# brain-research/l2hmc

Hardware: AMD Instinct MI355X
Metric: chain_leapfrog_steps_per_sec (higher is better)
Workload: dtype f32

## Files before the change

l2hmc_amd/csrc/l2hmc_abi.hip:

```cpp
#include <cstdlib>
#include "traj_tile.hpp"
#include "traj_lane.hpp"

namespace l2hmc {

thread_local char g_err[512] = "";
thread_local char g_kernel[96] = "";
void note_kernel(const char* fmt, long long a, long long b, long long c, long long d) { snprintf(g_kernel, sizeof(g_kernel), fmt, a, b, c, d); }

int fail(int code, const char* fmt, const char* a, long long b, long long c) {
  snprintf(g_err, sizeof(g_err), fmt, a, b, c);
  return code;
}

__global__ void pack_net_kernel(L2hmcNet net, int d, int H, int KH, int NT, float* out) {
  const int idx = blockIdx.x * blockDim.x + threadIdx.x;
  const int ngf = net_groups(NT) * 256;
  if (idx >= net_floats(NT)) return;
  float val = 0.f;
  if (idx < ngf) {
    const int g = idx >> 8, lane = (idx >> 2) & 63, r = idx & 3;
    const int i = lane & 15, q = lane >> 4;
    const int ui = ((i & 3) < KH) ? (i >> 2) * KH + (i & 3) : -1;
    const int uk = (r < KH) ? q * KH + r : -1;
// ... 292 lines not shown
  if (NW > 1 && (k.ekind == L2HMC_ENERGY_GAUSS_DENSE || k.ekind == L2HMC_ENERGY_GMM || lr))
    o += 16LL * k.xb_stride;
  k.o_red = (int)o;
  o += (long long)NW * 16 * 8;
  const int nc = k.ekind == L2HMC_ENERGY_GMM ? k.ncomp : 1;
  k.o_mu = (int)o;
  o += (long long)nc * DP;
  k.o_prec = (int)o;
  if (k.ekind == L2HMC_ENERGY_GAUSS_DIAG) o += DP;
  if ((k.ekind == L2HMC_ENERGY_GAUSS_DENSE || k.ekind == L2HMC_ENERGY_GMM) && !wg)
    o += (long long)nc * gauss_floats(NT);
  if (lr && NW > 1) o += (long long)NW * NT * 256;
  k.o_logc = (int)o;
  o += round4(nc);
  if (lr) {
    const long long need = logistic_floats(k.ncomp, k.d);
    const char* env = getenv("L2HMC_LOGISTIC_LDS");
    k.easy = !(env != nullptr && env[0] == '0') && (o + need + kLadLds) * 4 <= kMaxLdsBytes;
    if (k.easy) {
      k.o_mu = (int)o;
      o += need;
    }
  }
  return o * 4;
}

long long plan_lds_fast(KArgs& k, int NW, int DT, bool f16) {
  const int NT = k.NT, DP = 16 * NT, NTp = NW * DT;
  long long o = 0;
  k.o_fw = (int)o;
  o += 2LL * fast_fw_net(NTp, f16);
  k.o_fc = (int)o;
  o += 2LL * fast_fc_net(NTp);
  k.o_rec = (int)o;
  o += 2LL * fast_rec_dir(NTp, k.T);
  k.o_P = (int)o;
  if (NW > 1) o += 2LL * NW * 256;
  k.xb_stride = DP + 4;
  k.o_XB = (int)o;
  if (NW > 1 && (k.ekind == L2HMC_ENERGY_GAUSS_DENSE || k.ekind == L2HMC_ENERGY_GMM)) o += 16LL * k.xb_stride;
  k.o_red = (int)o;
  o += (long long)NW * 16 * 8;
  const int nc = k.ekind == L2HMC_ENERGY_GMM ? k.ncomp : 1;
  k.o_mu = (int)o;
  o += (long long)nc * DP;
  k.o_prec = (int)o;
  if (k.ekind == L2HMC_ENERGY_GAUSS_DIAG) o += DP;
  if (k.ekind == L2HMC_ENERGY_GAUSS_DENSE || k.ekind == L2HMC_ENERGY_GMM) o += (long long)nc * gauss_floats(NT);
  k.o_logc = (int)o;
  o += round4(nc);
  return o * 4;
}

long long plan_lds_tile(KArgs& k, int DT) {
  long long o = 0;
  k.o_fw = (int)o;
  o += 2LL * tile_fw_net(DT);
  k.o_state = (int)o;
  o += tile_l1_floats(DT);
  k.o_fc = (int)o;
  o += 2LL * fast_fc_net(DT);
  k.o_rec = (int)o;
  o += 2LL * fast_rec_dir(DT, k.T);
  k.o_mu = (int)o;
  o += 16LL * DT;
  k.o_prec = (int)o;
  o += 16LL * DT;
  k.o_logc = (int)o;
  return o * 4;
}

int check_energy(const L2hmcEnergy* e, int d) {
  if (e == nullptr) return fail(L2HMC_ERR_ARG, "energy is NULL%s");
  switch (e->kind) {
    case L2HMC_ENERGY_GAUSS_DIAG:
    case L2HMC_ENERGY_GAUSS_DENSE:
      if (!e->mu || !e->prec) return fail(L2HMC_ERR_ARG, "gaussian energy needs mu and prec%s");
      break;
    case L2HMC_ENERGY_GMM:
      if (!e->mu || !e->prec || !e->logc || e->n_comp < 1)
        return fail(L2HMC_ERR_ARG, "gmm energy needs mu, prec, logc, n_comp >= 1%s");
      break;
    case L2HMC_ENERGY_ROUGHWELL:
      if (!(e->eta > 0.f)) return fail(L2HMC_ERR_ARG, "roughwell needs eta > 0%s");
      break;
    case L2HMC_ENERGY_FUNNEL:
      if (!(e->eta > 0.f) || d < 2) return fail(L2HMC_ERR_ARG, "funnel needs sigma > 0 and d >= 2%s");
      break;
    case L2HMC_ENERGY_LOGISTIC:
      if (!e->mu) return fail(L2HMC_ERR_ARG, "logistic regression needs the packed data (mu, l2hmc_pack_logistic)%s");
      if (e->n_comp < 1 || e->n_comp > kLogisticMaxRows)
        return fail(L2HMC_ERR_ARG, "logistic regression needs 1 <= n_comp = n_data <= 1048576 (got %s%lld)", "", e->n_comp);
      if (d > kLogisticMaxDim) return fail(L2HMC_ERR_ARG, "logistic regression supports d <= 128 (got %s%lld)", "", d);
      if (!(e->eta > 0.f) || !(e->eta <= 3.402823466e38f))
        return fail(L2HMC_ERR_ARG, "logistic regression needs eta = prior variance sigma^2 > 0 and finite%s");
      break;
    default:
      return fail(L2HMC_ERR_ARG, "unknown energy kind %s%lld", "", e->kind);
  }
  if (!(e->temperature > 0.f)) return fail(L2HMC_ERR_ARG, "temperature must be > 0%s");
  if (!(e->anneal_beta >= 0.f && e->anneal_beta <= 1.f)) return fail(L2HMC_ERR_ARG, "anneal_beta must be in [0, 1] (0 = off)%s");
  return L2HMC_OK;
}

void fill_energy(KArgs& k, const L2hmcEnergy* e) {
  k.ekind = e->kind;
// ... 29 lines not shown
  if (v == 1) return false;
  NW = 4;
  DT = NT <= 8 ? 2 : (NT <= 16 ? 4 : 8);
  return NT <= 32;
}

bool pick_geometry_logistic(int d, int v, int& DT, int& NW) {
  if (d > kLogisticMaxDim || (v != 0 && v != 1 && v != 4)) return false;
  DT = tiles_of(d) <= 4 ? 1 : 2;
  NW = 4;
  if (v == 1) {
    DT = NW = 1;
    return tiles_of(d) <= 1;
  }
  return v == 0 || DT == 1;
}
bool pick_geometry_of(int ekind, int d, long long N, int v, int& DT, int& NW, int cus = 0) {
  return ekind == L2HMC_ENERGY_LOGISTIC ? pick_geometry_logistic(d, v, DT, NW) : pick_geometry(d, N, v, DT, NW, cus);
}

struct EnvOverrides {
  bool f32_mfma;
  int lane_res;
};

static EnvOverrides read_env() {
  static const bool f32 = [] { const char* e = getenv("L2HMC_F32_MFMA"); return e && e[0] && e[0] != '0'; }();
  const char* e = getenv("L2HMC_LANE_RES");
  return {f32, (e != nullptr && e[0] >= '0' && e[0] <= '2') ? e[0] - '0' : -1};
}

struct Variant {
  int value;
  int forced;
  bool all_auto;
  int geom;
  bool f32;
};

static Variant decode_variant(int variant, bool env_f32) {
  Variant v;
  v.f32 = variant >= 200 || env_f32;
  v.value = variant >= 200 ? variant - 200 : variant;
  v.forced = v.value >= 100 ? FAM_GENERAL : v.value == 32 ? FAM_LANE : v.value == 8 ? FAM_WIDE : v.value == 16 ? FAM_TILE : -1;
  v.all_auto = v.value == 0;
  v.geom = v.value >= 100 ? v.value - 100 : (v.value == 16 || v.value == 33) ? 0 : v.value;
  return v;
}

#ifndef WIDE_DENSE_MIN_NT
#define WIDE_DENSE_MIN_NT 8
#endif

static int plan_geometry(const L2hmcTrajectoryArgs& a, const Variant& v, int cus, TrajPlan& p) {
  if (!pick_geometry_of(a.energy.kind, a.d, a.n_chains, v.geom, p.DT, p.NW, cus))
    return fail(L2HMC_ERR_UNSUPPORTED, "d = %s%lld not supported with variant %lld", "", a.d, v.value);
  return L2HMC_OK;
}

static void plan_general(const L2hmcTrajectoryArgs& a, KArgs& k, TrajPlan& p) {
  p.family = FAM_GENERAL;
  p.lds = plan_lds(k, a.packed_nets != nullptr, true, p.NW, p.DT);
}

static int plan_trajectory(const L2hmcTrajectoryArgs& a, KArgs& k, int KH, int cus, const EnvOverrides& env, TrajPlan& p) {
  const Variant v = decode_variant(a.variant, env.f32_mfma);
  p = TrajPlan();
  p.ek = k.ekind;
  p.KH = KH <= 3 ? 3 : 4;
  const bool nets = a.packed_nets != nullptr, has_u = a.u != nullptr || (a.rng_flags & L2HMC_RNG_U);
  const bool plain = k.beta == 1.f && k.temperature == 1.f;
  const bool lr = k.ekind == L2HMC_ENERGY_LOGISTIC;
  if (lr && (v.forced == FAM_LANE || v.forced == FAM_WIDE || v.forced == FAM_TILE))
    return fail(L2HMC_ERR_UNSUPPORTED, "variant %s%lld: the logistic-regression target runs on the general kernel only (variant 0 or 100 + v)",
                "", v.value);
  if (lr) {
    int rc = plan_geometry(a, v, cus, p);
    if (rc) return rc;
    plan_general(a, k, p);
    return L2HMC_OK;
  }
  const bool lane_able = nets && a.ais_beta == nullptr && plain && k.n_steps >= 1 && lane_supported(k.ekind, a.d, a.H, k.ncomp) &&
                         (a.d <= 16 || a.x_next != nullptr || !has_u);
  if (v.forced == FAM_LANE && !lane_able)
    return fail(L2HMC_ERR_UNSUPPORTED, "variant 32 (one chain per lane) needs S/T/Q nets and a Gaussian / mixture / Rough-Well target with d <= 4%s");
  const bool lane_auto = (a.d <= 2 && a.n_chains >= 256 * cus) || (a.d <= 4 && a.n_chains >= 512 * cus);
  if (lane_able && (v.forced == FAM_LANE || (v.all_auto && lane_auto))) {
    p.family = FAM_LANE;
    p.DP = a.d <= 2 ? 2 : 4;
    p.HPR = lane_hu(a.H) == 10 ? 5 : 8;
    if (p.DP == 2 && p.HPR == 5)
      p.RES = env.lane_res >= 0 ? env.lane_res
              : k.ekind == L2HMC_ENERGY_GAUSS_DIAG ? 2
              : a.n_chains < 3LL * 64 * 1024 ? 1 : 0;
    return L2HMC_OK;
  }
  const bool wide_dense = k.ekind == L2HMC_ENERGY_GAUSS_DENSE || k.ekind == L2HMC_ENERGY_GMM;
  const bool wide_kind = k.ekind == L2HMC_ENERGY_GAUSS_DIAG || k.ekind == L2HMC_ENERGY_ROUGHWELL || wide_dense;
  const bool wide_able = nets && wide_kind && !(k.M > 1 && a.x_next == nullptr) && k.NT <= 32;
  if (v.forced == FAM_WIDE && !(wide_able && k.NT >= 4))
    return fail(L2HMC_ERR_UNSUPPORTED, "variant 8 (LDS-resident state) needs S/T/Q nets, a Gaussian or Rough-Well target, 64 <= d <= 512 and x_next when n_proposals > 1%s");
  if (wide_able && (v.forced == FAM_WIDE || (v.all_auto && k.NT > (wide_dense ? WIDE_DENSE_MIN_NT : 8)))) {
    KArgs kw = k;
    if (v.f32 || wide_dense || !plain) kw.packed16 = nullptr;
    int nw;
    const long long lds = plan_lds_wide(kw, nw);
    if (lds <= kMaxLdsBytes) {
      k = kw;
      p.family = FAM_WIDE;
      p.NW = nw;
      p.KH = KH == 3 ? 3 : 4;
      p.f16 = kw.packed16 != nullptr;
      p.lds = lds;
      return L2HMC_OK;
    }
    if (v.forced == FAM_WIDE) return fail(L2HMC_ERR_UNSUPPORTED, "variant 8: %s%lld bytes of LDS needed (T x d too large)", "", lds);
  }
  int rc = plan_geometry(a, v, cus, p);
  if (rc) return rc;
  const bool fast = nets && p.DT <= 2 && k.n_steps >= 1 && v.forced != FAM_GENERAL && plain;
  if (fast && a.d <= 4 && v.geom == 0 && k.ekind != L2HMC_ENERGY_FUNNEL && (k.ekind != L2HMC_ENERGY_GMM || k.ncomp <= 8)) {
    const long long lds = plan_lds_fast(k, 1, 1, !v.f32);
    if (lds <= kMaxLdsBytes) {
      p.family = FAM_SMALL;
      p.f16 = !v.f32;
      p.lds = lds;
      return L2HMC_OK;
    }
  }
  const bool tile_kind = k.ekind == L2HMC_ENERGY_GAUSS_DIAG || k.ekind == L2HMC_ENERGY_ROUGHWELL;
  const bool tileable = nets && tile_kind && k.NT >= 3 && k.NT <= 4 && k.n_steps >= 1 && plain && !(has_u && a.x_next == nullptr) &&
                        !v.f32;
  if (v.forced == FAM_TILE && !tileable)
    return fail(L2HMC_ERR_UNSUPPORTED, "variant 16 (one wave per tile) needs S/T/Q nets, a diagonal-Gaussian or Rough-Well target, 33 <= d <= 64 and x_next whenever u is given%s");
  if (tileable && (v.forced == FAM_TILE || (v.all_auto && a.n_chains >= 64LL * cus))) {
    const long long lds = plan_lds_tile(k, k.NT);
    if (lds <= kMaxLdsBytes) {
      p.family = FAM_TILE;
      p.DT = k.NT;
      p.tpw = (2 * lds > kMaxLdsBytes && a.n_chains >= 128LL * cus) ? 8 : 4;
      p.half = a.d - 16 * (k.NT - 1) <= 2;
      p.lds = lds;
      return L2HMC_OK;
    }
    if (v.forced == FAM_TILE)
      return fail(L2HMC_ERR_UNSUPPORTED, "variant 16: %s%lld bytes of LDS needed (T too large for the one-wave-per-tile kernel)", "", lds);
  }
  if (fast) {
    p.family = FAM_FAST;
    if (!v.f32 && tile_kind) {
      p.lds = plan_lds_fast(k, p.NW, p.DT, true);
      if (p.lds <= kMaxLdsBytes) {
        p.f16 = 1;
        return L2HMC_OK;
      }
    }
    p.lds = plan_lds_fast(k, p.NW, p.DT);
    if (p.lds <= kMaxLdsBytes) return L2HMC_OK;
  }
  plan_general(a, k, p);
  return L2HMC_OK;
}

static void note_plan(const TrajPlan& p) {
  switch (p.family) {
    case FAM_LANE:
      if (p.RES != 0) return note_kernel("traj_lane_kernel<%lld, %lld, %lld, %lld>", p.ek, p.DP, p.HPR, p.RES);
      return note_kernel("traj_lane_kernel<%lld, %lld, %lld>", p.ek, p.DP, p.HPR);
    case FAM_WIDE: return note_kernel(p.f16 ? "traj_wide_kernel<f16x2>" : "traj_wide_kernel");
    case FAM_SMALL: return note_kernel(p.f16 ? "traj_small_kernel<%lld, %lld, 1>" : "traj_small_kernel<%lld, %lld>", p.ek, p.KH);
    case FAM_TILE:
      return note_kernel(p.half ? "traj_tile_kernel<%lld, %lld, %lld, %lld, true>" : "traj_tile_kernel<%lld, %lld, %lld, %lld, false>",
                         p.ek, p.DT, p.KH, p.tpw);
    case FAM_FAST:
      return note_kernel(p.f16 ? "traj_fast_kernel<%lld, %lld, %lld, %lld, 1>" : "traj_fast_kernel<%lld, %lld, %lld, %lld>", p.ek, p.DT,
                         p.NW, p.KH);
    case FAM_LADDER: return note_kernel("traj_ladder_kernel<%lld, %lld, %lld, %lld>", p.ek, p.DT, p.NW, p.KH);
    default: return note_kernel("traj_kernel<%lld, %lld, %lld, %lld>", p.ek, p.DT, p.NW, p.KH);
  }
}

static int launch_plan(const TrajPlan& p, const KArgs& k, hipStream_t s, const LadArgs* lg = nullptr) {
  return on_energy_kind(p.ek, [&](auto ek) {
    constexpr int EK = decltype(ek)::value;
    if (p.family == FAM_LADDER) return launch_ladder_ek<EK>(p, k, *lg, s);
    if constexpr (EK != L2HMC_ENERGY_FUNNEL && EK != L2HMC_ENERGY_LOGISTIC) {
      if (p.family == FAM_LANE) return launch_lane_ek<EK>(p, k, s);
      if (p.family == FAM_WIDE) return launch_wide_ek<EK>(p, k, s);
    }
    if constexpr (EK == L2HMC_ENERGY_GAUSS_DIAG || EK == L2HMC_ENERGY_ROUGHWELL) {
      if (p.family == FAM_TILE) return launch_tile_ek<EK>(p, k, s);
      if (p.family == FAM_FAST && p.f16) return launch_fast16_ek<EK>(p, k, s);
    }
    return launch_ek<EK>(p, k, s);
  });
}

}

using namespace l2hmc;

#ifdef L2HMC_PHASE_TIMING
static unsigned long long* g_dbg = nullptr;
extern "C" void l2hmc_set_debug_buffer(void* p) { g_dbg = (unsigned long long*)p; }
#define L2HMC_DBG_PTR g_dbg
#else
#define L2HMC_DBG_PTR nullptr
#endif

extern "C" {

int l2hmc_abi_version(void) { return L2HMC_ABI_VERSION; }

int32_t l2hmc_last_kernel(char* buf, int32_t n) {
  if (!buf || n < 1) return fail(L2HMC_ERR_ARG, "l2hmc_last_kernel: bad argument%s");
  snprintf(buf, (size_t)n, "%s", g_kernel);
  return (int32_t)strlen(g_kernel);
}

const char* l2hmc_last_error(void) { return g_err; }

int64_t l2hmc_struct_bytes(int32_t which) {
  switch (which) {
    case L2HMC_STRUCT_NET: return sizeof(L2hmcNet);
    case L2HMC_STRUCT_ENERGY: return sizeof(L2hmcEnergy);
    case L2HMC_STRUCT_TRAJECTORY_ARGS: return sizeof(L2hmcTrajectoryArgs);
    case L2HMC_STRUCT_MLP3: return sizeof(L2hmcMlp3);
    case L2HMC_STRUCT_SPLIT_ARGS: return sizeof(L2hmcSplitArgs);
    case L2HMC_STRUCT_TRAIN_ARGS: return sizeof(L2hmcTrainArgs);
    case L2HMC_STRUCT_TRAIN_SPLIT_ARGS: return sizeof(L2hmcTrainSplitArgs);
    case L2HMC_STRUCT_TRAIN_STEP: return sizeof(L2hmcTrainStep);
    case L2HMC_STRUCT_LADDER_ARGS: return sizeof(L2hmcLadderArgs);
  }
  return fail(L2HMC_ERR_ARG, "l2hmc_struct_bytes: unknown struct id%s");
}

int64_t l2hmc_packed_nets_floats(int32_t d, int32_t H) {
  if (d < 1 || H < 1) return fail(L2HMC_ERR_ARG, "d and H must be >= 1%s");
  if (H > 15) return fail(L2HMC_ERR_UNSUPPORTED, "fused nets support H <= 15 (got %s%lld)", "", H);
  if (d > 512) return fail(L2HMC_ERR_UNSUPPORTED, "fused nets support d <= 512 (got %s%lld)", "", d);
  return 2LL * net_floats(tiles_of(d)) + 2LL * lane_layout(d, H).total + 2LL * net_f16_floats(tiles_of(d));
// ... 365 lines not shown
```

l2hmc_amd/csrc/l2hmc_kernels.hpp:

```cpp
#pragma once
#include <hip/hip_runtime.h>
#include <stdint.h>
#include <stdio.h>
#include <string.h>
#include <type_traits>

#include "../../include/l2hmc.h"

namespace l2hmc {

typedef float f4 __attribute__((ext_vector_type(4)));

#define MFMA16(a, b, c) __builtin_amdgcn_mfma_f32_16x16x4f32((a), (b), (c), 0, 0, 0)

__host__ __device__ constexpr bool weights_in_global(int DT) { return DT >= 4; }

int fail(int code, const char* fmt, const char* a = "", long long b = 0, long long c = 0);
inline float roughwell_den(const L2hmcEnergy* e) {
  if (e->den > 0.f) return e->den;
  return e->easy ? e->eta : (float)((double)e->eta * (double)e->eta);
}
void note_kernel(const char* fmt, long long a = 0, long long b = 0, long long c = 0, long long d = 0);
inline bool adam_args_ok(float lr, float beta1, float beta2, float epsilon, int64_t step) {
  return step >= 1 && lr >= 0.f && (beta1 >= 0.f && beta1 < 1.f) && (beta2 >= 0.f && beta2 < 1.f) && epsilon > 0.f;
// ... 854 lines not shown
  extern __shared__ __attribute__((aligned(16))) float smem[];
  lds_poison(smem);
  const int tid = threadIdx.x, lane = tid & 63;
  const int w = NW > 1 ? __builtin_amdgcn_readfirstlane(tid >> 6) : 0;
  const int c = lane & 15, q = lane >> 4;
  const long long chain = (long long)blockIdx.x * 16 + c;
  const bool live = chain < A.N;
  stage_energy<EK, weights_in_global(DT)>(A, smem, tid, 64 * NW);
  f4 x[DT], g[DT];
  load_state<DT, NW>(A.x, A, chain, live, w, q, x);
  __syncthreads();
  float U[1];
  grad_energy<EK, DT, NW>(A, smem, w, lane, x, g, U[0], true);
  store_state<DT, NW>(A.grad_out, A, chain, live, w, q, g);
  chain_allreduce<NW, 1>(U, smem + A.o_red, w, lane);
  if (A.U_out != nullptr && live && w == 0 && lane < 16) A.U_out[chain] = U[0];
}

template <int EK, int DT, int NW>
__global__ __launch_bounds__(64 * NW) void paccept_kernel(const KArgs A) {
  extern __shared__ __attribute__((aligned(16))) float smem[];
  lds_poison(smem);
  const int tid = threadIdx.x, lane = tid & 63;
  const int w = NW > 1 ? __builtin_amdgcn_readfirstlane(tid >> 6) : 0;
  const int c = lane & 15, q = lane >> 4;
  const long long chain = (long long)blockIdx.x * 16 + c;
  const bool live = chain < A.N;
  stage_energy<EK, weights_in_global(DT)>(A, smem, tid, 64 * NW);
  f4 x[DT], v[DT], g[DT];
  float red[4];
  __syncthreads();
  load_state<DT, NW>(A.x, A, chain, live, w, q, x);
  load_state<DT, NW>(A.v, A, chain, live, w, q, v);
  grad_energy<EK, DT, NW>(A, smem, w, lane, x, g, red[0], true);
  red[1] = 0.f;
#pragma unroll
  for (int t = 0; t < DT; ++t) red[1] += 0.5f * hsum(v[t] * v[t]);
  load_state<DT, NW>(A.x1, A, chain, live, w, q, x);
  load_state<DT, NW>(A.v1, A, chain, live, w, q, v);
  grad_energy<EK, DT, NW>(A, smem, w, lane, x, g, red[2], true);
  red[3] = 0.f;
#pragma unroll
  for (int t = 0; t < DT; ++t) red[3] += 0.5f * hsum(v[t] * v[t]);
  chain_allreduce<NW, 4>(red, smem + A.o_red, w, lane);
  if (live && w == 0 && lane < 16) {
    const float val = (red[0] + red[1]) - (red[2] + red[3]) + A.logjac_in[chain];
    A.p_out[chain] = accept_prob(val);
  }
}


const int kMaxLdsBytes = 160 * 1024;

enum Family { FAM_GENERAL, FAM_FAST, FAM_SMALL, FAM_TILE, FAM_WIDE, FAM_LANE, FAM_LADDER, FAM_ENERGY, FAM_PACCEPT };

struct TrajPlan {
  int family = FAM_GENERAL;
  int ek = 0;
  int DT = 1, NW = 1;
  int KH = 3;
  int tpw = 4;
  bool half = false;
  int DP = 0, HPR = 0, RES = 0;
  int f16 = 0;
  long long lds = 0;
};

template <class K, class... X>
int launch_kernel(K kern, long long blocks, int threads, long long lds_bytes, hipStream_t s, const X&... args) {
  if (lds_bytes > kMaxLdsBytes)
    return fail(L2HMC_ERR_UNSUPPORTED, "needs %s%lld bytes of LDS (> 160 KiB): d too large for the LDS-resident weight path", "", lds_bytes);
  if (lds_bytes > 48 * 1024) {
    hipError_t e = hipFuncSetAttribute(reinterpret_cast<const void*>(kern),
                                       hipFuncAttributeMaxDynamicSharedMemorySize, (int)lds_bytes);
    if (e != hipSuccess) return fail(L2HMC_ERR_HIP, "hipFuncSetAttribute: %s", hipGetErrorString(e));
  }
  if (blocks > 0x7fffffffLL) return fail(L2HMC_ERR_UNSUPPORTED, "too many chains%s");
  hipLaunchKernelGGL(kern, dim3((unsigned)blocks), dim3(threads), (size_t)lds_bytes, s, args...);
  hipError_t e = hipGetLastError();
  if (e != hipSuccess) return fail(L2HMC_ERR_HIP, "kernel launch: %s", hipGetErrorString(e));
  return L2HMC_OK;
}

template <auto V> using ic = std::integral_constant<decltype(V), V>;

template <auto A, auto B, class F>
int on_either(bool first, F&& f) { return first ? f(ic<A>{}) : f(ic<B>{}); }

template <class F>
int on_energy_kind(int ek, F&& f) {
  switch (ek) {
    case 1: return f(ic<1>{});
    case 2: return f(ic<2>{});
    case 3: return f(ic<3>{});
    case 4: return f(ic<4>{});
    case 5: return f(ic<5>{});
    case 7: return f(ic<7>{});
  }
  return fail(L2HMC_ERR_ARG, "unknown energy kind%s");
}

template <int DT_, int NW_> struct Geom { static constexpr int DT = DT_, NW = NW_; };
template <class... G> struct Geoms {};
using GeneralGeoms = Geoms<Geom<1, 1>, Geom<2, 1>, Geom<4, 1>, Geom<1, 4>, Geom<2, 4>, Geom<4, 4>, Geom<8, 4>>;
using LogisticGeoms = Geoms<Geom<1, 1>, Geom<1, 4>, Geom<2, 4>>;
using FastGeoms = Geoms<Geom<1, 1>, Geom<2, 1>, Geom<1, 4>, Geom<2, 4>, Geom<2, 2>>;

template <class... G, class F>
int on_geometry(Geoms<G...>, int DT, int NW, const char* what, F&& f) {
  int rc = L2HMC_OK;
  const bool found = ((DT == G::DT && NW == G::NW && ((rc = f(ic<G::DT>{}, ic<G::NW>{})), true)) || ...);
  return found ? rc : fail(L2HMC_ERR_UNSUPPORTED, "no %skernel for this geometry", what);
}

template <int EK>
int launch_ek(const TrajPlan& p, const KArgs& k, hipStream_t s);
template <int EK>
int launch_fast16_ek(const TrajPlan& p, const KArgs& k, hipStream_t s);
template <int EK>
int launch_tile_ek(const TrajPlan& p, const KArgs& k, hipStream_t s);
template <int EK>
int launch_ladder_ek(const TrajPlan& p, const KArgs& k, const LadArgs& l, hipStream_t s);
template <int EK>
int launch_wide_ek(const TrajPlan& p, const KArgs& k, hipStream_t s);
template <int EK>
int launch_lane_ek(const TrajPlan& p, const KArgs& k, hipStream_t s);

}
```

l2hmc_amd/csrc/traj_fast.hpp:

```cpp
#pragma once
#include "l2hmc_kernels.hpp"
#include "bf3k.hpp"


namespace l2hmc {

__device__ __forceinline__ float relu_i(float a) { return __int_as_float(max(__float_as_int(a), 0)); }
__device__ __forceinline__ f4 rcp4(f4 a) {
  return f4{__builtin_amdgcn_rcpf(a.x), __builtin_amdgcn_rcpf(a.y), __builtin_amdgcn_rcpf(a.z),
            __builtin_amdgcn_rcpf(a.w)};
}
__device__ __forceinline__ f4 ex2_4(f4 a) {
  return f4{__builtin_amdgcn_exp2f(a.x), __builtin_amdgcn_exp2f(a.y), __builtin_amdgcn_exp2f(a.z),
            __builtin_amdgcn_exp2f(a.w)};
}

typedef _Float16 h2v __attribute__((ext_vector_type(2)));
typedef _Float16 h8v __attribute__((ext_vector_type(8)));
typedef float f2v __attribute__((ext_vector_type(2)));
#define L2HMC_F16_SCALE 64.0f
struct WF16 {
  h8v a1;
  h8v a2;
};
// ... 2 lines not shown
  h2v r;
  const float ns = -L2HMC_F16_SCALE;
  asm("v_fma_mixlo_f16 %0, %1, %2, %3 op_sel:[0,0,0] op_sel_hi:[1,0,0]" : "=v"(r) : "v"(h), "s"(ns), "v"(a0));
  asm("v_fma_mixhi_f16 %0, %1, %2, %3 op_sel:[1,0,0] op_sel_hi:[1,0,0]" : "+v"(r) : "v"(h), "s"(ns), "v"(a1));
  return r;
}
template <bool LAT>
__device__ __forceinline__ h8v split16(f4 a) {
  const f4 ad = a * (1.f / L2HMC_F16_SCALE);
  const h2v h01 = cvt_pk16(ad.x, ad.y), h23 = cvt_pk16(ad.z, ad.w);
  h2v l01, l23;
  if constexpr (LAT) {
    float r0, r1, r2, r3;
    const float ns = -L2HMC_F16_SCALE;
    asm("v_fma_mix_f32 %0, %1, %2, %3 op_sel:[0,0,0] op_sel_hi:[1,0,0]" : "=v"(r0) : "v"(h01), "s"(ns), "v"(a.x));
    asm("v_fma_mix_f32 %0, %1, %2, %3 op_sel:[1,0,0] op_sel_hi:[1,0,0]" : "=v"(r1) : "v"(h01), "s"(ns), "v"(a.y));
    asm("v_fma_mix_f32 %0, %1, %2, %3 op_sel:[0,0,0] op_sel_hi:[1,0,0]" : "=v"(r2) : "v"(h23), "s"(ns), "v"(a.z));
    asm("v_fma_mix_f32 %0, %1, %2, %3 op_sel:[1,0,0] op_sel_hi:[1,0,0]" : "=v"(r3) : "v"(h23), "s"(ns), "v"(a.w));
    l01 = cvt_pk16(r0, r1);
    l23 = cvt_pk16(r2, r3);
  } else {
    l01 = lo_pair16(h01, a.x, a.y);
    l23 = lo_pair16(h23, a.z, a.w);
  }
  return h8v{h01.x, h01.y, h23.x, h23.y, l01.x, l01.y, l23.x, l23.y};
}
__device__ __forceinline__ WF16 wsplit16(f4 w) {
  const float sc = L2HMC_F16_SCALE;
  const h2v h01 = cvt_pk16(w.x, w.y), h23 = cvt_pk16(w.z, w.w);
  const f4 r = f4{w.x - (float)h01.x, w.y - (float)h01.y, w.z - (float)h23.x, w.w - (float)h23.y} * sc;
  const h2v L01 = cvt_pk16(r.x, r.y), L23 = cvt_pk16(r.z, r.w);
  const h2v H01 = cvt_pk16((float)h01.x * sc, (float)h01.y * sc), H23 = cvt_pk16((float)h23.x * sc, (float)h23.y * sc);
  const h2v l01 = cvt_pk16((float)L01.x / sc, (float)L01.y / sc), l23 = cvt_pk16((float)L23.x / sc, (float)L23.y / sc);
  WF16 f;
  f.a1 = h8v{H01.x, H01.y, H23.x, H23.y, h01.x, h01.y, h23.x, h23.y};
  f.a2 = h8v{L01.x, L01.y, L23.x, L23.y, l01.x, l01.y, l23.x, l23.y};
  return f;
}
#define L2HMC_F16_STATE_MAX 2.5e5f
__device__ __forceinline__ float amax4(f4 a) { return fmaxf(fmaxf(fabsf(a.x), fabsf(a.y)), fmaxf(fabsf(a.z), fabsf(a.w))); }
__device__ __forceinline__ f4 mfma16x2(const WF16& W, h8v b, f4 acc) {
  acc = __builtin_amdgcn_mfma_f32_16x16x32_f16(W.a1, b, acc, 0, 0, 0);
  return __builtin_amdgcn_mfma_f32_16x16x32_f16(W.a2, b, acc, 0, 0, 0);
}

__host__ __device__ constexpr int fast_fw_net_f32(int NTp) { return (3 * NTp + 1) * 256; }
__host__ __device__ constexpr int fast_fw_net(int NTp, bool f16 = false) { return (3 * NTp + 1) * (f16 ? 512 : 256); }
__host__ __device__ inline int fast_dpp(int NTp) { return 16 * NTp + 16; }
__host__ __device__ inline int fast_fc_net(int NTp) { return 4 * fast_dpp(NTp); }
__host__ __device__ inline int fast_rec(int NTp) { return 32 + 16 * NTp; }
__host__ __device__ inline int fast_rec_dir(int NTp, int T) { return (T + 2) * fast_rec(NTp) + 16; }

long long plan_lds_fast(KArgs& k, int NW, int DT, bool f16 = false);

#ifndef L2HMC_FAST_SPLIT_LAT_TAIL
#define L2HMC_FAST_SPLIT_LAT_TAIL true
#endif
#ifndef L2HMC_FAST_SPLIT_LAT_PAIR
#define L2HMC_FAST_SPLIT_LAT_PAIR true
#endif
#ifndef L2HMC_FAST_SPLIT_LAT_L1
#define L2HMC_FAST_SPLIT_LAT_L1 false
#endif
template <int DT, bool F16 = false>
struct TailK {
  f4 w2;
  f4 hs[DT], ht[DT], hq[DT];
  f4 cS[DT], cQ[DT], bQ[DT];
};
template <int DT>
struct TailK<DT, true> {
  WF16 w2;
  WF16 hs[DT], ht[DT], hq[DT];
  f4 cS[DT], cQ[DT], bQ[DT];
};

template <int DT>
__device__ __forceinline__ void load_tailk(TailK<DT, false>& tk, const float* fw, const float* fc, int dofs, int NTp,
                                           int w, int lane) {
  const int q = lane >> 4, DPp = fast_dpp(NTp);
  tk.w2 = lds4(fw + lane * 4);
#pragma unroll
  for (int t = 0; t < DT; ++t) {
    const int tg = w * DT + t;
    tk.hs[t] = lds4(fw + ((1 + 3 * tg + 0) * 64 + lane) * 4);
    tk.ht[t] = lds4(fw + ((1 + 3 * tg + 1) * 64 + lane) * 4);
    tk.hq[t] = lds4(fw + ((1 + 3 * tg + 2) * 64 + lane) * 4);
    tk.cS[t] = lds4(fc + dofs + 16 * tg + 4 * q);
    tk.cQ[t] = lds4(fc + 2 * DPp + 16 * tg + 4 * q);
    tk.bQ[t] = lds4(fc + 3 * DPp + 16 * tg + 4 * q);
  }
}
__device__ __forceinline__ WF16 lds_wf16(const float* fw, int NTp, int g, int lane) {
  WF16 f;
  f.a1 = *reinterpret_cast<const h8v*>(fw + (g * 64 + lane) * 4);
  f.a2 = *reinterpret_cast<const h8v*>(fw + (3 * NTp + 1) * 256 + (g * 64 + lane) * 4);
  return f;
}
template <int DT>
__device__ __forceinline__ void load_tailk(TailK<DT, true>& tk, const float* fw, const float* fc, int dofs, int NTp,
                                           int w, int lane) {
  const int q = lane >> 4, DPp = fast_dpp(NTp);
  tk.w2 = lds_wf16(fw, NTp, 0, lane);
#pragma unroll
  for (int t = 0; t < DT; ++t) {
    const int tg = w * DT + t;
// ... 496 lines not shown
```

Before: 2.381 billion.

## Add eight-wave half-tile fast kernel for diagonal-Gaussian mid-size chain counts

Adds a new trajectory kernel in which eight waves each handle half of a 16-dimension tile (two dims per lane) for the diagonal Gaussian with f16x2 MFMA. The planner picks it automatically over the four-wave fast kernel when chain counts are moderate (at least 1024 and at most 16 per CU), doubling waves per block to raise parallelism when there are too few chains to fill the GPU. In exchange it adds more cross-wave exchanges through LDS and a larger LDS footprint, and it only applies when d lies between 33 and 64.

```diff
diff --git a/l2hmc_amd/csrc/l2hmc_abi.hip b/l2hmc_amd/csrc/l2hmc_abi.hip
--- a/l2hmc_amd/csrc/l2hmc_abi.hip
+++ b/l2hmc_amd/csrc/l2hmc_abi.hip
@@ -368,6 +368,30 @@
   return o * 4;
 }
 
+long long plan_lds_fast8(KArgs& k) {
+  const int NT = k.NT, DP = 16 * NT, NTp = 4, NW = 8;
+  long long o = 0;
+  k.o_fw = (int)o;
+  o += 2LL * fast_fw_net(NTp, true);
+  k.o_fc = (int)o;
+  o += 2LL * fast_fc_net(NTp);
+  k.o_rec = (int)o;
+  o += 2LL * fast_rec_dir(NTp, k.T);
+  k.o_P = (int)o;
+  o += 2LL * NW * 256;
+  k.xb_stride = DP + 4;
+  k.o_XB = (int)o;
+  k.o_red = (int)o;
+  o += (long long)NW * 16 * 8;
+  k.o_mu = (int)o;
+  o += DP;
+  k.o_prec = (int)o;
+  o += DP;
+  k.o_logc = (int)o;
+  o += 4;
+  return o * 4;
+}
+
 long long plan_lds_tile(KArgs& k, int DT) {
   long long o = 0;
   k.o_fw = (int)o;
@@ -503,6 +527,10 @@
 #define WIDE_DENSE_MIN_NT 8
 #endif
 
+#ifndef FAST8_MIN_CHAINS
+#define FAST8_MIN_CHAINS 1024
+#endif
+
 static int plan_geometry(const L2hmcTrajectoryArgs& a, const Variant& v, int cus, TrajPlan& p) {
   if (!pick_geometry_of(a.energy.kind, a.d, a.n_chains, v.geom, p.DT, p.NW, cus))
     return fail(L2HMC_ERR_UNSUPPORTED, "d = %s%lld not supported with variant %lld", "", a.d, v.value);
@@ -529,6 +557,20 @@
     int rc = plan_geometry(a, v, cus, p);
     if (rc) return rc;
     plan_general(a, k, p);
+    return L2HMC_OK;
+  }
+  const bool fast8_able = nets && k.ekind == L2HMC_ENERGY_GAUSS_DIAG && k.NT >= 3 && k.NT <= 4 && k.n_steps >= 1 && plain && !v.f32;
+  if (v.value == 7) {
+    if (v.f32) return fail(L2HMC_ERR_UNSUPPORTED, "variant 7 (eight half-tile waves per tile) has no f32-input form (variant 207 / L2HMC_F32_MFMA)%s");
+    if (!fast8_able)
+      return fail(L2HMC_ERR_UNSUPPORTED, "variant 7 (eight half-tile waves per tile) needs S/T/Q nets, a diagonal-Gaussian target, 33 <= d <= 64 and n_steps >= 1%s");
+    const long long lds = plan_lds_fast8(k);
+    if (lds > kMaxLdsBytes) return fail(L2HMC_ERR_UNSUPPORTED, "variant 7: %s%lld bytes of LDS needed (T too large)", "", lds);
+    p.family = FAM_FAST8;
+    p.DT = 1;
+    p.NW = 8;
+    p.f16 = 1;
+    p.lds = lds;
     return L2HMC_OK;
   }
   const bool lane_able = nets && a.ais_beta == nullptr && plain && k.n_steps >= 1 && lane_supported(k.ekind, a.d, a.H, k.ncomp) &&
@@ -598,6 +640,18 @@
       return fail(L2HMC_ERR_UNSUPPORTED, "variant 16: %s%lld bytes of LDS needed (T too large for the one-wave-per-tile kernel)", "", lds);
   }
   if (fast) {
+    if (fast8_able && v.geom == 0 && v.forced == -1 && p.NW == 4 && p.DT == 1 && a.n_chains >= FAST8_MIN_CHAINS && a.n_chains <= 16LL * cus) {
+      KArgs k8 = k;
+      const long long lds = plan_lds_fast8(k8);
+      if (lds <= kMaxLdsBytes) {
+        k = k8;
+        p.family = FAM_FAST8;
+        p.NW = 8;
+        p.f16 = 1;
+        p.lds = lds;
+        return L2HMC_OK;
+      }
+    }
     p.family = FAM_FAST;
     if (!v.f32 && tile_kind) {
       p.lds = plan_lds_fast(k, p.NW, p.DT, true);
@@ -626,6 +680,7 @@
     case FAM_FAST:
       return note_kernel(p.f16 ? "traj_fast_kernel<%lld, %lld, %lld, %lld, 1>" : "traj_fast_kernel<%lld, %lld, %lld, %lld>", p.ek, p.DT,
                          p.NW, p.KH);
+    case FAM_FAST8: return note_kernel("traj_fast8_kernel<%lld, %lld, 1>", p.ek, p.KH);
     case FAM_LADDER: return note_kernel("traj_ladder_kernel<%lld, %lld, %lld, %lld>", p.ek, p.DT, p.NW, p.KH);
     default: return note_kernel("traj_kernel<%lld, %lld, %lld, %lld>", p.ek, p.DT, p.NW, p.KH);
   }
@@ -638,6 +693,9 @@
     if constexpr (EK != L2HMC_ENERGY_FUNNEL && EK != L2HMC_ENERGY_LOGISTIC) {
       if (p.family == FAM_LANE) return launch_lane_ek<EK>(p, k, s);
       if (p.family == FAM_WIDE) return launch_wide_ek<EK>(p, k, s);
+    }
+    if constexpr (EK == L2HMC_ENERGY_GAUSS_DIAG) {
+      if (p.family == FAM_FAST8) return launch_fast8_ek<EK>(p, k, s);
     }
     if constexpr (EK == L2HMC_ENERGY_GAUSS_DIAG || EK == L2HMC_ENERGY_ROUGHWELL) {
       if (p.family == FAM_TILE) return launch_tile_ek<EK>(p, k, s);
diff --git a/l2hmc_amd/csrc/l2hmc_kernels.hpp b/l2hmc_amd/csrc/l2hmc_kernels.hpp
--- a/l2hmc_amd/csrc/l2hmc_kernels.hpp
+++ b/l2hmc_amd/csrc/l2hmc_kernels.hpp
@@ -930,7 +930,7 @@
 
 const int kMaxLdsBytes = 160 * 1024;
 
-enum Family { FAM_GENERAL, FAM_FAST, FAM_SMALL, FAM_TILE, FAM_WIDE, FAM_LANE, FAM_LADDER, FAM_ENERGY, FAM_PACCEPT };
+enum Family { FAM_GENERAL, FAM_FAST, FAM_SMALL, FAM_TILE, FAM_WIDE, FAM_LANE, FAM_LADDER, FAM_ENERGY, FAM_PACCEPT, FAM_FAST8 };
 
 struct TrajPlan {
   int family = FAM_GENERAL;
@@ -996,6 +996,8 @@
 template <int EK>
 int launch_fast16_ek(const TrajPlan& p, const KArgs& k, hipStream_t s);
 template <int EK>
+int launch_fast8_ek(const TrajPlan& p, const KArgs& k, hipStream_t s);
+template <int EK>
 int launch_tile_ek(const TrajPlan& p, const KArgs& k, hipStream_t s);
 template <int EK>
 int launch_ladder_ek(const TrajPlan& p, const KArgs& k, const LadArgs& l, hipStream_t s);
diff --git a/l2hmc_amd/csrc/traj_fast.hpp b/l2hmc_amd/csrc/traj_fast.hpp
--- a/l2hmc_amd/csrc/traj_fast.hpp
+++ b/l2hmc_amd/csrc/traj_fast.hpp
@@ -78,6 +78,7 @@
 __host__ __device__ inline int fast_rec_dir(int NTp, int T) { return (T + 2) * fast_rec(NTp) + 16; }
 
 long long plan_lds_fast(KArgs& k, int NW, int DT, bool f16 = false);
+long long plan_lds_fast8(KArgs& k);
 
 #ifndef L2HMC_FAST_SPLIT_LAT_TAIL
 #define L2HMC_FAST_SPLIT_LAT_TAIL true
diff --git a/l2hmc_amd/csrc/traj_fast8.hip b/l2hmc_amd/csrc/traj_fast8.hip
--- /dev/null
+++ b/l2hmc_amd/csrc/traj_fast8.hip
@@ -0,0 +1,11 @@
+#include "traj_fast8.hpp"
+
+namespace l2hmc {
+
+template <int EK>
+int launch_fast8_ek(const TrajPlan& p, const KArgs& k, hipStream_t s) {
+  return on_either<3, 4>(p.KH == 3, [&](auto KH) { return launch_kernel(traj_fast8_kernel<EK, KH, 1>, (k.N + 15) / 16, 512, p.lds, s, k); });
+}
+
+template int launch_fast8_ek<1>(const TrajPlan& p, const KArgs& k, hipStream_t s);
+}
diff --git a/l2hmc_amd/csrc/traj_fast8.hpp b/l2hmc_amd/csrc/traj_fast8.hpp
--- /dev/null
+++ b/l2hmc_amd/csrc/traj_fast8.hpp
@@ -0,0 +1,426 @@
+#pragma once
+#include "traj_fast.hpp"
+
+namespace l2hmc {
+
+__device__ __forceinline__ f2v lds2(const float* p) { return *reinterpret_cast<const f2v*>(p); }
+__device__ __forceinline__ f2v splat2(float a) { return f2v{a, a}; }
+__device__ __forceinline__ f2v ex2_2(f2v a) { return f2v{__builtin_amdgcn_exp2f(a.x), __builtin_amdgcn_exp2f(a.y)}; }
+__device__ __forceinline__ float hsum2(f2v a) { return a.x + a.y; }
+__device__ __forceinline__ float amax2(f2v a) { return fmaxf(fabsf(a.x), fabsf(a.y)); }
+__device__ __forceinline__ f2v sel2(bool c, f2v a, f2v b) { return c ? a : b; }
+__device__ __forceinline__ f2v half_of(f4 a, int hf) { return hf ? f2v{a.z, a.w} : f2v{a.x, a.y}; }
+
+__device__ __forceinline__ h8v split16h(f2v a) {
+  const f2v ad = a * (1.f / L2HMC_F16_SCALE);
+  const h2v h = cvt_pk16(ad.x, ad.y);
+  const h2v l = lo_pair16(h, a.x, a.y);
+  const _Float16 z = (_Float16)0.f;
+  return h8v{h.x, h.y, z, z, l.x, l.y, z, z};
+}
+
+#ifndef L2HMC_FAST8_SPLIT_LAT
+#define L2HMC_FAST8_SPLIT_LAT false
+#endif
+
+constexpr int kFast8NTp = 4;
+
+struct TailK8 {
+  WF16 w2, hsq, ht;
+  f2v cS, cQ, bQ;
+};
+__device__ __forceinline__ void load_tailk8(TailK8& tk, const float* fw, const float* fc, int dofs, int tg, int hf, int lane) {
+  const int q = lane >> 4, DPp = fast_dpp(kFast8NTp);
+  const int src = (lane & 0x3c) + 2 * hf + (lane & 1);
+  const bool upper = (lane & 2) != 0;
+  tk.w2 = lds_wf16(fw, kFast8NTp, 0, lane);
+  tk.hsq = lds_wf16(fw, kFast8NTp, 1 + 3 * tg + (upper ? 2 : 0), src);
+  tk.ht = lds_wf16(fw, kFast8NTp, 1 + 3 * tg + 1, src);
+  if (upper) {
+    const _Float16 z = (_Float16)0.f;
+    tk.ht.a1 = h8v{z, z, z, z, z, z, z, z};
+    tk.ht.a2 = tk.ht.a1;
+  }
+  const int dim = 16 * tg + 4 * q + 2 * hf;
+  tk.cS = lds2(fc + dofs + dim);
+  tk.cQ = lds2(fc + 2 * DPp + dim);
+  tk.bQ = lds2(fc + 3 * DPp + dim);
+}
+
+template <int KH, class F>
+__device__ __forceinline__ void tail_fast8(const TailK8& tk, f4 hs_, F&& apply) {
+  f4 h = splat(0.f);
+#pragma unroll
+  for (int r = 0; r < KH; ++r) h[r] = relu_i(hs_[r]);
+  {
+    const f4 acc = mfma16x2(tk.w2, split16<L2HMC_FAST8_SPLIT_LAT>(h), splat(0.f));
+#pragma unroll
+    for (int r = 0; r < KH; ++r) h[r] = relu_i(acc[r]);
+  }
+  const h8v b = split16<L2HMC_FAST8_SPLIT_LAT>(h);
+  f4 zsq = __builtin_amdgcn_mfma_f32_16x16x32_f16(tk.hsq.a1, b, splat(0.f), 0, 0, 0);
+  f4 zt = __builtin_amdgcn_mfma_f32_16x16x32_f16(tk.ht.a1, b, splat(0.f), 0, 0, 0);
+  zsq = __builtin_amdgcn_mfma_f32_16x16x32_f16(tk.hsq.a2, b, zsq, 0, 0, 0);
+  zt = __builtin_amdgcn_mfma_f32_16x16x32_f16(tk.ht.a2, b, zt, 0, 0, 0);
+  const f4 r = rcp4(-(ex2_4(zsq) * 0.5f + 0.5f));
+  const f2v aS = f2v{r.x, r.y} * tk.cS + tk.cS;
+  const f2v EQ = ex2_2(f2v{r.z, r.w} * tk.cQ + tk.bQ);
+  apply(aS, f2v{zt.x, zt.y}, EQ);
+}
+
+template <int KH, class FA, class FB>
+__device__ __forceinline__ void tail_fast8_2(const TailK8& tk, f4 hsa, f4 hsb, FA&& applyA, FB&& keepB) {
+  f4 ha = splat(0.f), hb = splat(0.f);
+#pragma unroll
+  for (int r = 0; r < KH; ++r) { ha[r] = relu_i(hsa[r]); hb[r] = relu_i(hsb[r]); }
+  {
+    const h8v sa = split16<L2HMC_FAST8_SPLIT_LAT>(ha), sb = split16<L2HMC_FAST8_SPLIT_LAT>(hb);
+    f4 acca = __builtin_amdgcn_mfma_f32_16x16x32_f16(tk.w2.a1, sa, splat(0.f), 0, 0, 0);
+    f4 accb = __builtin_amdgcn_mfma_f32_16x16x32_f16(tk.w2.a1, sb, splat(0.f), 0, 0, 0);
+    acca = __builtin_amdgcn_mfma_f32_16x16x32_f16(tk.w2.a2, sa, acca, 0, 0, 0);
+    accb = __builtin_amdgcn_mfma_f32_16x16x32_f16(tk.w2.a2, sb, accb, 0, 0, 0);
+#pragma unroll
+    for (int r = 0; r < KH; ++r) { ha[r] = relu_i(acca[r]); hb[r] = relu_i(accb[r]); }
+  }
+  const h8v ba = split16<L2HMC_FAST8_SPLIT_LAT>(ha), bb = split16<L2HMC_FAST8_SPLIT_LAT>(hb);
+  f4 zsqa = __builtin_amdgcn_mfma_f32_16x16x32_f16(tk.hsq.a1, ba, splat(0.f), 0, 0, 0);
+  f4 zta = __builtin_amdgcn_mfma_f32_16x16x32_f16(tk.ht.a1, ba, splat(0.f), 0, 0, 0);
+  f4 zsqb = __builtin_amdgcn_mfma_f32_16x16x32_f16(tk.hsq.a1, bb, splat(0.f), 0, 0, 0);
+  f4 ztb = __builtin_amdgcn_mfma_f32_16x16x32_f16(tk.ht.a1, bb, splat(0.f), 0, 0, 0);
+  zsqa = __builtin_amdgcn_mfma_f32_16x16x32_f16(tk.hsq.a2, ba, zsqa, 0, 0, 0);
+  zta = __builtin_amdgcn_mfma_f32_16x16x32_f16(tk.ht.a2, ba, zta, 0, 0, 0);
+  zsqb = __builtin_amdgcn_mfma_f32_16x16x32_f16(tk.hsq.a2, bb, zsqb, 0, 0, 0);
+  ztb = __builtin_amdgcn_mfma_f32_16x16x32_f16(tk.ht.a2, bb, ztb, 0, 0, 0);
+  const f4 ra = rcp4(-(ex2_4(zsqa) * 0.5f + 0.5f));
+  const f2v aSa = f2v{ra.x, ra.y} * tk.cS + tk.cS;
+  const f2v EQa = ex2_2(f2v{ra.z, ra.w} * tk.cQ + tk.bQ);
+  applyA(aSa, f2v{zta.x, zta.y}, EQa);
+  const f4 rb = rcp4(-(ex2_4(zsqb) * 0.5f + 0.5f));
+  const f2v aSb = f2v{rb.x, rb.y} * tk.cS + tk.cS;
+  const f2v EQb = ex2_2(f2v{rb.z, rb.w} * tk.cQ + tk.bQ);
+  keepB(aSb, f2v{ztb.x, ztb.y}, EQb);
+}
+
+__device__ __forceinline__ f2v load_state8(const float* p, const KArgs& A, long long chain, bool live, int dim0) {
+  f2v r = splat2(0.f);
+  if (live && p != nullptr) {
+    const float* row = p + chain * A.d + dim0;
+    if ((A.d & 1) == 0) {
+      if (dim0 < A.d) r = *reinterpret_cast<const f2v*>(row);
+    } else {
+      if (dim0 + 0 < A.d) r.x = row[0];
+      if (dim0 + 1 < A.d) r.y = row[1];
+    }
+  }
+  return r;
+}
+__device__ __forceinline__ void store_state8(float* p, const KArgs& A, long long chain, bool live, int dim0, f2v z) {
+  if (p == nullptr || !live) return;
+  float* row = p + chain * A.d + dim0;
+  if ((A.d & 1) == 0) {
+    if (dim0 < A.d) *reinterpret_cast<f2v*>(row) = z;
+  } else {
+    if (dim0 + 0 < A.d) row[0] = z.x;
+    if (dim0 + 1 < A.d) row[1] = z.y;
+  }
+}
+
+__device__ __forceinline__ f4 l1_half16(f2v z, f4 acc, const WF16& W) { return mfma16x2(W, split16h(z), acc); }
+
+#ifndef L2HMC_FAST8_SERIAL_TAILS
+#define L2HMC_FAST8_PAIR true
+#else
+#define L2HMC_FAST8_PAIR false
+#endif
+
+template <int EK, int KH, int PK = 1>
+__global__ __launch_bounds__(512, 2) void traj_fast8_kernel(const KArgs A) {
+  extern __shared__ __attribute__((aligned(16))) float smem[];
+  lds_poison(smem);
+  static_assert(EK == L2HMC_ENERGY_GAUSS_DIAG && PK == 1, "the eight-wave kernel serves the diagonal Gaussian as f16x2");
+  constexpr int NW = 8, NTp = kFast8NTp;
+  const int tid = threadIdx.x, lane = tid & 63, nthr = 64 * NW;
+  const int w8 = __builtin_amdgcn_readfirstlane(tid >> 6);
+  const int tg = w8 >> 1, hf = w8 & 1;
+  const int c = lane & 15, q = lane >> 4;
+  const int dim4 = 16 * tg + 4 * q, dim0 = dim4 + 2 * hf;
+  const long long chain = (long long)blockIdx.x * 16 + c;
+  const bool live = chain < A.N;
+  const int NT = A.NT, DP = 16 * NT, NF = net_floats(NT);
+  const float LOG2E = 1.4426950408889634f;
+  const float eps = A.alpha != nullptr ? expf(*A.alpha) : A.eps_host;
+  const float heps = 0.5f * eps;
+  const int FWN = fast_fw_net(NTp, true), DPp = fast_dpp(NTp), FCN = fast_fc_net(NTp), R = fast_rec(NTp),
+            RECD = fast_rec_dir(NTp, A.T);
+
+  {
+    constexpr int GN = 3 * NTp + 1;
+    constexpr int NCP = 2 * GN * 64, NTRIP = (NCP + 64 * NW - 1) / (64 * NW);
+    for (int t0 = 0; t0 < NTRIP; t0 += 4) {
+      f4 buf[4];
+#pragma unroll
+      for (int u = 0; u < 4; ++u) {
+        const int i = tid + (t0 + u) * nthr;
+        const int net = i >= GN * 64, j = i - net * (GN * 64), g = j >> 6;
+        buf[u] = splat(0.f);
+        if (i < NCP && g < 3 * NT + 1) buf[u] = reinterpret_cast<const f4*>(A.packed + (size_t)net * NF + (2 * NT + 1) * 256)[j];
+      }
+#pragma unroll
+      for (int u = 0; u < 4; ++u) {
+        const int i = tid + (t0 + u) * nthr;
+        const int net = i >= GN * 64, j = i - net * (GN * 64), g = j >> 6;
+        float sc = 1.f;
+        if (g > 0) sc = ((g - 1) % 3 == 1) ? (net == 0 ? eps : heps) : 2.f * LOG2E;
+        if (i < NCP) {
+          const WF16 f = wsplit16(buf[u] * sc);
+          float* base = smem + A.o_fw + net * FWN;
+          reinterpret_cast<h8v*>(base)[j] = f.a1;
+          reinterpret_cast<h8v*>(base + GN * 256)[j] = f.a2;
+        }
+      }
+    }
+  }
+  for (int i = tid; i < 2 * 16 * NTp; i += nthr) {
+    const int net = i / (16 * NTp), dim = i % (16 * NTp);
+    const float* scl = A.packed + (size_t)net * NF + net_groups(NT) * 256;
+    const float epn = net == 0 ? eps : heps;
+    const float es = dim < DP ? scl[dim] : 0.f, eq = dim < DP ? scl[DP + dim] : 0.f;
+    const float cs = es * epn * LOG2E, cq = eq * eps * LOG2E;
+    float* fc = smem + A.o_fc + net * FCN;
+    fc[dim] = cs;
+    fc[DPp + dim] = -cs;
+    fc[2 * DPp + dim] = cq;
+    fc[3 * DPp + dim] = cq + log2f(epn);
+  }
+#pragma unroll 4
+  for (int i = tid; i < 2 * A.T * R; i += nthr) {
+    const int dr = i / (A.T * R), r = (i / R) % A.T, j = i % R;
+    const bool tb = j < 32;
+    const int net = tb ? j >> 4 : 0, u = j & 15, dim = tb ? 0 : j - 32;
+    const float* tf = A.packed + (size_t)net * NF + (2 * NT * 64) * 4;
+    const float a0 = tf[u * 4], a1 = tf[(16 + u) * 4], a2 = tf[(32 + u) * 4], c0 = A.trig[2 * r], c1 = A.trig[2 * r + 1];
+    const float mk = A.masks[r * A.d + (dim < A.d ? dim : 0)];
+    const float m = dim < A.d ? mk : 0.f;
+    smem[A.o_rec + dr * RECD + (r + 1) * R + j] = tb ? fmaf(a0, c0, fmaf(a1, c1, a2)) : (dr ? m : 1.f - m);
+  }
+  stage_energy<EK, false>(A, smem, tid, nthr);
+
+  f2v x = load_state8(A.x, A, chain, live, dim0), v, g;
+  const bool need_p = A.p_out != nullptr || A.x_next != nullptr || A.u != nullptr ||
+                      (A.rng_flags & L2HMC_RNG_U) != 0;
+  __syncthreads();
+
+  const float* fwx = smem + A.o_fw;
+  const float* fwv = fwx + FWN;
+  const float* fcx = smem + A.o_fc;
+  const float* fcv = fcx + FCN;
+  int pb = 0;
+  const f4 Z = splat(0.f);
+  const bool tile_ok = tg < NT;
+  const f4 mu4 = tile_ok ? lds4(smem + A.o_mu + dim4) : Z, prec4 = tile_ok ? lds4(smem + A.o_prec + dim4) : Z;
+  const f2v mu = half_of(mu4, hf), prec = half_of(prec4, hf);
+  auto diag_U = [&](f2v xx, f2v gg) { return 0.5f * hsum2((xx - mu) * gg); };
+  g = prec * (x - mu);
+  float U_start = diag_U(x, g);
+
+  WF16 l1xa, l1xb, l1va;
+  f4 pv[1];
+  {
+    const bool ok = 16 * tg < A.d;
+    const float* wx = A.packed;
+    const float* wv = A.packed + NF;
+    const f4 xa = ok ? lds4(wx + (tg * 64 + lane) * 4) : Z, xb = ok ? lds4(wx + ((NT + tg) * 64 + lane) * 4) : Z;
+    f4 va = ok ? lds4(wv + (tg * 64 + lane) * 4) : Z;
+    const f4 vb = ok ? lds4(wv + ((NT + tg) * 64 + lane) * 4) : Z;
+    va = va + prec4 * vb;
+    const f4 pm4 = -(prec4 * mu4);
+    const f4 pmh = hf ? f4{0.f, 0.f, pm4.z, pm4.w} : f4{pm4.x, pm4.y, 0.f, 0.f};
+    f4 cv[1] = {Z};
+#pragma unroll
+    for (int r = 0; r < 4; ++r) cv[0] = MFMA16(vb[r], pmh[r], cv[0]);
+    xchg<NW, 1>(cv, A, smem, w8, lane, pb);
+    if (w8 == 0 && c == 0) {
+      for (int i = 0; i < 2 * A.T; ++i) {
+        float* tb = smem + A.o_rec + (i / A.T) * RECD + (i % A.T + 1) * R + 16 + 4 * q;
+        *reinterpret_cast<f4*>(tb) = lds4(tb) + cv[0];
+      }
+    }
+    __syncthreads();
+    const f2v xah = half_of(xa, hf), xbh = half_of(xb, hf), vah = half_of(va, hf);
+    l1xa = wsplit16(f4{xah.x, xah.y, 0.f, 0.f});
+    l1xb = wsplit16(f4{xbh.x, xbh.y, 0.f, 0.f});
+    l1va = wsplit16(f4{vah.x, vah.y, 0.f, 0.f});
+  }
+  PT_DECL;
+  PT_MARK(0);
+  pv[0] = l1_half16(x, Z, l1va);
+  xchg<NW, 1>(pv, A, smem, w8, lane, pb);
+
+  const long long gchain = A.chain_off + chain;
+  const bool rng_v = (A.rng_flags & L2HMC_RNG_V) != 0, rng_d = (A.rng_flags & L2HMC_RNG_DIR) != 0;
+  const bool rng_u = (A.rng_flags & L2HMC_RNG_U) != 0;
+  f2v vn = splat2(0.f);
+  if (!rng_v) vn = load_state8(A.v, A, chain, live, dim0);
+  bool fwd_n = (A.dir != nullptr && !rng_d) ? (live ? A.dir[chain] != 0 : true) : (A.dir_all != 0);
+  float u_n = (A.u != nullptr && !rng_u && live) ? A.u[chain] : 0.f;
+  const bool have_u = A.u != nullptr || rng_u;
+  for (int m = 0; m < A.M; ++m) {
+    const long long moff = (long long)m * A.N;
+    const unsigned long long prop = A.rng_prop0 + (unsigned long long)m;
+    if (rng_v) {
+      const f2v n = half_of(philox_normal4(A.rng_seed, gchain, (unsigned)(dim4 >> 2), prop), hf);
+      v = f2v{dim0 + 0 < A.d ? n.x : 0.f, dim0 + 1 < A.d ? n.y : 0.f};
+    } else {
+      v = vn;
+    }
+    bool fwd = fwd_n;
+    float u_m = u_n;
+    if (rng_d || rng_u) {
+      bool fr;
+      float ur;
+      philox_dir_u(A.rng_seed, gchain, prop, fr, ur);
+      if (rng_d) fwd = fr;
+      if (rng_u) u_m = ur;
+    }
+    if (m + 1 < A.M) {
+      if (!rng_v) vn = load_state8(A.v + (moff + A.N) * A.d, A, chain, live, dim0);
+      if (A.dir != nullptr && !rng_d && live) fwd_n = A.dir[moff + A.N + chain] != 0;
+      if (A.u != nullptr && !rng_u && live) u_n = A.u[moff + A.N + chain];
+    }
+    const f2v x0 = x;
+    const f4 pv0 = pv[0];
+    float red[6];
+    float amax_l = fmaxf(amax2(x), fmaxf(amax2(v), amax2(g)));
+    red[0] = U_start;
+    red[1] = 0.5f * hsum2(v * v);
+    red[2] = 0.f;
+    f2v ldv = splat2(0.f);
+
+    const float ff = fwd ? 1.f : 0.f, nf = ff - 1.f;
+    const int dofs = fwd ? 0 : DPp;
+    const int row0 = fwd ? A.step_begin : (A.T - 1 - A.step_begin);
+    const float* rec = smem + A.o_rec + (fwd ? RECD : 0) + (row0 + 1) * R + 4 * q;
+    const int drec = fwd ? R : -R;
+    f4 tbv = lds4(rec + 16);
+
+    TailK8 tkx, tk;
+    load_tailk8(tkx, fwx, fcx, dofs, tg, hf, lane);
+    load_tailk8(tk, fwv, fcv, dofs, tg, hf, lane);
+    constexpr bool PAIR = L2HMC_FAST8_PAIR;
+    f2v aS_n, T_n, EQ_n;
+    if constexpr (PAIR) {
+      tail_fast8<KH>(tk, pv[0] + tbv, [&](f2v aS, f2v T, f2v EQ) { aS_n = aS; T_n = T; EQ_n = EQ; });
+    }
+    for (int it = 0; it < A.n_steps; ++it) {
+      f2v vh, y, xin;
+      const f4 tbx = lds4(rec);
+      const f2v k1 = lds2(rec + 32 + 16 * tg + 2 * hf);
+      rec += drec;
+      const f4 tbv_n = lds4(rec + 16);
+
+      PT_MARK(1);
+      auto vhalf1 = [&](f2v aS, f2v T, f2v EQ) {
+        const f2v ES = ex2_2(aS);
+        ldv += aS;
+        const f2v tr = T - EQ * g;
+        vh = ES * (nf * tr + v) + ff * tr;
+      };
+      if constexpr (PAIR) vhalf1(aS_n, T_n, EQ_n);
+      else tail_fast8<KH>(tk, pv[0] + tbv, vhalf1);
+      PT_MARK(2);
+
+      xin = k1 * x;
+      f4 px[1];
+      const f4 pa = l1_half16(vh, Z, l1xa);
+      px[0] = l1_half16(xin, pa, l1xb);
+      PT_MARK(3);
+      xchg<NW, 1>(px, A, smem, w8, lane, pb);
+      PT_MARK(4);
+      tail_fast8<KH>(tkx, px[0] + tbx, [&](f2v aS, f2v T, f2v EQ) {
+        const f2v up = 1.f - k1;
+        const f2v aSm = up * aS;
+        const f2v ES = ex2_2(aSm);
+        ldv += aSm;
+        const f2v tr = up * (EQ * vh + T);
+        y = ES * (nf * tr + x) + ff * tr;
+        xin = up * y;
+      });
+      PT_MARK(5);
+      f4 py[1];
+      py[0] = l1_half16(xin, pa, l1xb);
+      PT_MARK(6);
+      xchg<NW, 1>(py, A, smem, w8, lane, pb);
+      PT_MARK(7);
+      tail_fast8<KH>(tkx, py[0] + tbx, [&](f2v aS, f2v T, f2v EQ) {
+        const f2v aSm = k1 * aS;
+        const f2v ES = ex2_2(aSm);
+        ldv += aSm;
+        const f2v tr = k1 * (EQ * vh + T);
+        x = ES * (nf * tr + y) + ff * tr;
+      });
+      PT_MARK(8);
+
+      g = prec * (x - mu);
+      pv[0] = l1_half16(x, Z, l1va);
+      PT_MARK(9);
+      xchg<NW, 1>(pv, A, smem, w8, lane, pb);
+      PT_MARK(10);
+      auto vhalf2 = [&](f2v aS, f2v T, f2v EQ) {
+        const f2v ES = ex2_2(aS);
+        ldv += aS;
+        const f2v tr = T - EQ * g;
+        v = ES * (nf * tr + vh) + ff * tr;
+      };
+      if constexpr (PAIR) {
+        tail_fast8_2<KH>(tk, pv[0] + tbv, pv[0] + tbv_n, vhalf2, [&](f2v aS, f2v T, f2v EQ) { aS_n = aS; T_n = T; EQ_n = EQ; });
+      } else {
+        tail_fast8<KH>(tk, pv[0] + tbv, vhalf2);
+      }
+      PT_MARK(11);
+      tbv = tbv_n;
+    }
+    red[2] = diag_U(x, g);
+    const float ld = hsum2(ldv) * 0.6931471805599453f;
+
+    const bool last = m == A.M - 1;
+    red[3] = 0.5f * hsum2(v * v);
+    red[4] = ld;
+    const float U_end = red[2];
+    amax_l = fmaxf(amax_l, fmaxf(amax2(x), fmaxf(amax2(v), amax2(g))));
+    red[5] = amax_l < L2HMC_F16_STATE_MAX ? 0.f : 1.f;
+    chain_allreduce<NW, 6>(red, smem + A.o_red, w8, lane);
+    if (red[5] > 0.f) {
+      const float qnan = __uint_as_float(0x7fc00000u);
+      x = splat2(qnan);
+      v = splat2(qnan);
+      red[4] = qnan;
+    }
+    if (last) {
+      store_state8(A.x_out, A, chain, live, dim0, x);
+      store_state8(A.v_out, A, chain, live, dim0, v);
+    }
+    const bool writer = live && w8 == 0 && lane < 16;
+    if (A.logjac_out != nullptr && writer) A.logjac_out[moff + chain] = red[4];
+    if (need_p) {
+      const float val = (red[0] + red[1]) - (red[2] + red[3]) + red[4];
+      const float p = accept_prob(val);
+      if (A.p_out != nullptr && writer) A.p_out[moff + chain] = p;
+      if (have_u) {
+        const bool acc = live && (p - u_m) >= 0.f;
+        x = sel2(acc, x, x0);
+        g = prec * (x - mu);
+        pv[0] = sel4(acc, pv[0], pv0);
+        U_start = acc ? U_end : U_start;
+      } else {
+        U_start = U_end;
+      }
+    } else {
+      U_start = U_end;
+    }
+    if (A.x_hist != nullptr) store_state8(A.x_hist + moff * A.d, A, chain, live, dim0, x);
+  }
+  PT_FLUSH(w8, lane);
+  store_state8(A.x_next, A, chain, live, dim0, x);
+}
+
+}
```

Result: slower. 1.668 billion (-30.0%).
